# ZhenlongYuan/TSAR-MVS

Hardware: AMD Instinct MI355X
Metric: depthmap Mpixels/sec (ETH3D full-res, 8 iters) (higher is better)
Workload: dtype f32

## Files before the change

tsar-mvs_amd/csrc/pm_core.h:

```cpp
#pragma once
#include <type_traits>

#include "tsar_device_math.h"

#define PM_BLOCK 256
#define PM_RW 32

#include "pm_tap_common.h"

template <bool QUAD, bool DIFF = false>
DEVFN float sample_bilinear(const DevView& vw, int w, int h, int qpitch, float u, float v, bool q8 = false) {
    u = fminf(fmaxf(u, -1.0f), (float)w);
    v = fminf(fmaxf(v, -1.0f), (float)h);
    const float fu = floorf(u), fv = floorf(v);
    float ax = u - fu, ay = v - fv;
    if (q8) { ax = rintf(ax * 256.0f) * 0.00390625f; ay = rintf(ay * 256.0f) * 0.00390625f; }
    const int iu = (int)fu, iv = (int)fv;
    float t00, t10, t01, t11;
    if (QUAD) {
        const uint32_t off = (uint32_t)(__mul24(iv + 1, qpitch) + iu + 1) * 4u;
        const uint32_t q = *(global_u32_ptr)((const char __attribute__((address_space(1)))*)vw.quad + off);
        t00 = (float)(q & 0xffu);
        t10 = (float)((q >> 8) & 0xffu);
        t01 = (float)((q >> 16) & 0xffu);
// ... 102 lines not shown
    const int w = sc->w, h = sc->h;
    const float xf = (float)x, yf = (float)y;
    const float xd = xf * D, yd = yf * D;
    const float a = ((vw.A[0] * xd + vw.A[1] * yd) + vw.A[2] * D) + vw.b[0];
    const float b = ((vw.A[3] * xd + vw.A[4] * yd) + vw.A[5] * D) + vw.b[1];
    const float s = ((vw.A[6] * xd + vw.A[7] * yd) + vw.A[8] * D) + vw.b[2];
    float u, v;
    persp_divide_exact<true>(a, b, s, u, v);
    const float cf = floorf(u + 0.5f), rf = floorf(v + 0.5f);
    const bool inside = s > 0.0f && cf >= 0.0f && cf <= (float)(w - 1) && rf >= 0.0f && rf <= (float)(h - 1);
    float Dv = 0.0f;
    if (inside) Dv = ((global_f32_ptr)dm)[(int)rf * w + (int)cf];
    const float* M = sc->geom_back[vi];
    const float cd = cf * Dv, rd = rf * Dv;
    const float p0 = ((M[0] * cd + M[1] * rd) + M[2] * Dv) + M[3];
    const float p1 = ((M[4] * cd + M[5] * rd) + M[6] * Dv) + M[7];
    const float p2 = ((M[8] * cd + M[9] * rd) + M[10] * Dv) + M[11];
    float xq, yq;
    persp_divide_exact<true>(p0, p1, p2, xq, yq);
    const float dx = xq - xf, dy = yq - yf;
    const float e2 = dx * dx + dy * dy;
    const float tau = sc->geom_clip;
    const float r = sqrt_rsq_exact(fminf(fmaxf(e2, 0x1p-100f), 0x1p100f));
    float e = e2 < 0x1p-100f ? 0.0f : r;
    e = (inside && Dv > 0.0f && p2 > 0.0f && e2 < sc->geom_clip_sq) ? fminf(e, tau) : tau;
    return sc->geom_weight * e;
}

DEVFN float add_prior_term(const DevScene* __restrict__ sc, int x, int y, const float4& n4, float D, float c) {
    const float4* pp = sc->prior;
    if (pp == nullptr) return c;
    typedef float prior_entry __attribute__((ext_vector_type(4)));
    const prior_entry q = ((const __attribute__((address_space(1))) prior_entry*)pp)[y * sc->w + x];
    const float Dp = q.w;
    const float a = fabsf(D - Dp);
    const float rel = a / Dp;
    const float dclip = sc->prior_depth_clip, nclip = sc->prior_normal_clip;
    const float r_d = rel < dclip ? rel / dclip : 1.0f;
    const float s = 1.0f - ((n4.x * q.x + n4.y * q.y) + n4.z * q.z);
    const float s0 = s < 0.0f ? 0.0f : s;
    const float r_n = s < nclip ? s0 / nclip : 1.0f;
    const float t = (sc->prior_weight_depth * r_d) + (sc->prior_weight_normal * r_n);
    return Dp > 0.0f ? c + t : c;
}

template <int NB, int HR, bool STRICT, bool QUAD, int V = 0, int BLK = PM_BLOCK>
DEVFN float multiview_cost(const DevScene* __restrict__ sc, const typename TileOf<QUAD>::type* tile, int tw, int own, const float* wts, const PixelRef& pr,
                           int x, int y, const float4& n4, int& beview, float& ratio, bool prune = false, float cost_now = 0.0f, int* skipped = nullptr) {
    constexpr bool GEOM = (V & TSAR_V_GEOM) != 0;
    constexpr bool PRUNE = (V & TSAR_V_PRUNE) != 0;
    static_assert(!PRUNE || !GEOM, "the bound speaks of the photometric cost alone");
    constexpr bool PAIR = (V & TSAR_V_PAIR) != 0;
    static_assert(!PAIR || (!PRUNE && !GEOM), "the paired gathers exist for the plain fast box-11 kernels");
    constexpr int VT = V & ~(TSAR_V_GEOM | TSAR_V_REDRAW | TSAR_V_PRUNE | TSAR_V_PAIR);
    float best[NB];
#pragma unroll
    for (int k = 0; k < NB; k++) best[k] = __builtin_inff();
    const int num = sc->n_sel;
    int valid = 0, bv = -1;
    float cmin = __builtin_inff();
    float depth_h = 0.0f;
    if constexpr (GEOM) depth_h = plane_depth(sc->ref, n4, x, y);
    int vi_next = sc->sel[0];
    for (int i = 0; i < num; i++) {
        const int vi = vi_next;
        vi_next = sc->sel[i + 1 < num ? i + 1 : i];
        float c;
        if constexpr ((VT & TSAR_V_LUT) != 0) c = view_cost_lut<STRICT, (VT >> 11) & 7, (VT & TSAR_V_BUF) != 0 && !STRICT, (VT & TSAR_V_MIX) != 0 && !STRICT>(sc, sc->view[vi], tile, tw, own, wts, pr, x, y, n4);
        else if constexpr (QUAD && HR == 5 && r5_production_variant(VT) && PRUNE) {
            static_assert((VT & 250) == 250 && !STRICT, "pruning instantiations exist for the fast row-wise loop");
            ViewPrune vp;
            vp.on = prune; vp.skipped = false;
            vp.cost_now = cmin < cost_now ? TSAR_MAXCOST : cost_now;
            c = view_cost_r5<false, true, true, (VT & TSAR_V_BUF) != 0, (VT & TSAR_V_MIX) != 0, BLK, 0, true>(sc, sc->view[vi], tile, tw, own, wts, pr, x, y, n4, &vp);
            if (vp.skipped) *skipped += 1;
        } else if constexpr (QUAD && HR == 5 && PAIR && VT == 250) {
            static_assert(!STRICT, "the paired gathers exist for the fast row-wise loop");
            c = view_cost_r5<false, true, true, false, false, BLK, 0, false, true>(sc, sc->view[vi], tile, tw, own, wts, pr, x, y, n4);
        } else if constexpr (QUAD && HR == 5 && r5_production_variant(VT))
            c = view_cost_r5<STRICT, (VT & 128) != 0 && !STRICT, (VT & 8) != 0, (VT & TSAR_V_BUF) != 0, (VT & TSAR_V_MIX) != 0, BLK>(sc, sc->view[vi], tile, tw, own, wts, pr, x, y, n4);
#ifdef TSAR_EXPERIMENTS
        else if constexpr (QUAD && HR == 5 && PAIR && VT == (250 | 4194304))
            c = view_cost_r5<false, true, true, false, false, BLK, 3, false, true>(sc, sc->view[vi], tile, tw, own, wts, pr, x, y, n4);
        else if constexpr (QUAD && HR == 5 && r5_diag_variant(VT))
            c = view_cost_r5<false, true, true, true, true, BLK, (VT & 4194304) ? 1 : 2>(sc, sc->view[vi], tile, tw, own, wts, pr, x, y, n4);
#endif
        else {
            static_assert(VT == 0, "unknown tap-loop variant");
            c = view_cost_generic<HR, STRICT, QUAD, BLK>(sc, sc->view[vi], tile, tw, own, wts, pr, x, y, n4);
        }
        auto vmin = [](float a, float b) { float r; asm("v_min_f32 %0, %1, %2" : "=v"(r) : "v"(a), "v"(b)); return r; };
        auto vmax = [](float a, float b) { float r; asm("v_max_f32 %0, %1, %2" : "=v"(r) : "v"(a), "v"(b)); return r; };
        c = vmin(c, TSAR_MAXCOST);
        valid -= (int32_t)__float_as_uint(c - TSAR_MAXCOST) >> 31;
        if constexpr (GEOM) c = c + geom_term(sc, sc->view[vi], vi, x, y, depth_h);
        {
            const uint32_t worse = (uint32_t)((int32_t)__float_as_uint(cmin - c) >> 31);
            asm("v_bfi_b32 %0, %1, %2, %3" : "=v"(bv) : "v"(worse), "v"(bv), "s"(vi));
            cmin = vmin(cmin, c);
        }
        float v = c;
#pragma unroll
        for (int k = 0; k < NB; k++) {
            const float lo = vmin(best[k], v), hi = vmax(best[k], v);
            best[k] = lo;
            v = hi;
        }
    }
    int nb = valid;
    if (sc->cost_comb == TSAR_COMB_BEST_N) nb = min(nb, sc->n_best);
    if (nb <= 0) { beview = -1; ratio = 0.f; return TSAR_MAXCOST; }
    float cost = 0.f;
#pragma unroll
    for (int k = 0; k < NB; k++)
        if (k < nb) cost += best[k];
    cost = cost / (float)nb;
    ratio = num >= 2 ? best[0] / best[1] : 0.f;
    beview = bv;
    if constexpr (GEOM) cost = add_prior_term(sc, x, y, n4, depth_h, cost);
    return cost;
}

DEVFN void strip_tile(int t, int tiles_x, int tiles_y, int sw, int& tx, int& ty) {
    if (sw <= 0) { ty = t / tiles_x; tx = t - ty * tiles_x; return; }
    const int per_strip = sw * tiles_y;
    const int strip = t / per_strip, within = t - strip * per_strip;
    const int width = min(sw, tiles_x - strip * sw);
    ty = within / width;
    tx = strip * sw + within - ty * width;
}

static inline int strip_width(int requested, int tiles_x) {
    if (requested >= 0) return requested;
// ... 10 lines not shown
```

tsar-mvs_amd/csrc/pm_sweep.hip:

```cpp
#include "pm_sweep_impl.h"

__global__ void d16_probe_kernel(uint32_t* out) {
    __shared__ unsigned short t[64];
    t[threadIdx.x] = (unsigned short)(0x4300u + threadIdx.x);
    __syncthreads();
    uint32_t r = 0xffffffffu;
    const uint32_t addr = (uint32_t)(uintptr_t)(const __attribute__((address_space(3))) unsigned short*)(t + threadIdx.x);
    asm volatile("ds_read_u16_d16_hi %0, %1\n\ts_waitcnt lgkmcnt(0)" : "+v"(r) : "v"(addr));
    out[threadIdx.x] = r;
}
bool probe_d16_hi_zeroes(tsar_ctx* ctx) {
    CallFrame f(ctx, "d16 probe", nullptr, false);
    uint32_t h[64];
    uint32_t* d = f.out(h, 64, TSAR_MEM_HOST);
    if (f.ok()) {
        hipLaunchKernelGGL(d16_probe_kernel, dim3(1), dim3(64), 0, ctx->stream, d);
        f.launched();
    }
    bool ok = f.finish() == TSAR_OK;
    for (int i = 0; ok && i < 64; i++) ok = h[i] == ((0x4300u + i) << 16);
    return ok;
}

template <int NB, int HR>
static int launch_sweep_nh(tsar_ctx* ctx, int colour, const PlaneBuf& a, const PlaneBuf& b, const PlaneBuf& c, uint32_t sid, int dp, int dr) {
    const bool strict = ctx->hscene.flags & TSAR_FLAG_STRICT_DIV, quad = ctx->hscene.use_quad;
    const bool buf = ctx->buffer_gather && ctx->sweeps_done >= (strict ? (ctx->buffer_from > 2 ? ctx->buffer_from : 2) : ctx->buffer_from);
    const int v = ctx->variant;
    if constexpr ((NB == 2 || NB == 4) && HR == 5)
    if (quad && !(ctx->hscene.flags & TSAR_FLAG_TEX_FILTER_8BIT) && (v == 250 || v == 122 || (v == 114 && NB == 2))) {
#define SWEEP_R5(S, V, B) (buf ? launch_sweep_g<NB, 5, S, true, (V) | TSAR_V_BUF, B>(ctx, colour, a, b, c, sid, dp, dr) : launch_sweep_g<NB, 5, S, true, V, B>(ctx, colour, a, b, c, sid, dp, dr))
        const bool mix = buf && !strict && v == 250 && ctx->hscene.n_sel > 0 && ctx->hscene.view[ctx->hscene.sel[0]].dquad != nullptr;
#define SWEEP_R5_FAST250_ALL(B) (mix ? launch_sweep_g<NB, 5, false, true, 250 | TSAR_V_BUF | TSAR_V_MIX, B>(ctx, colour, a, b, c, sid, dp, dr) : SWEEP_R5(false, 250, B))
        const bool prune = NB == 2 && !strict && v == 250 && ctx->prune && ctx->prune_steps > 0 && dr && ctx->call_launch >= ctx->prune_from &&
                           ctx->hscene.cost_comb == TSAR_COMB_BEST_N && ctx->hscene.n_best == 1 && !scene_has_terms(ctx->hscene);
#define SWEEP_R5_PRUNE(B) (mix ? launch_sweep_t<2, 5, false, true, 250 | TSAR_V_BUF | TSAR_V_MIX | TSAR_V_PRUNE, B>(ctx, colour, a, b, c, sid, dp, dr) \
                           : buf ? launch_sweep_t<2, 5, false, true, 250 | TSAR_V_BUF | TSAR_V_PRUNE, B>(ctx, colour, a, b, c, sid, dp, dr)              \
                                 : launch_sweep_t<2, 5, false, true, 250 | TSAR_V_PRUNE, B>(ctx, colour, a, b, c, sid, dp, dr))
        const bool pair = NB == 2 && !strict && v == 250 && !buf && !prune && (ctx->pair & 2) && !scene_has_terms(ctx->hscene);
#define SWEEP_R5_FAST250(B) (prune ? SWEEP_R5_PRUNE(B) : pair ? launch_pm_sweep_pair(ctx, B, colour, a, b, c, sid, dp, dr) : SWEEP_R5_FAST250_ALL(B))
        if constexpr (NB == 2) {
            const int tiles256 = ((ctx->hscene.w + PM_RW - 1) / PM_RW) * ((ctx->hscene.h + 15) / 16);
            bool small = tiles256 < SWEEP_SMALL_IMAGE_TILES;
            if (ctx->force_block) small = ctx->force_block == 128;
            if (small && v != 114) {
                if (strict) return SWEEP_R5(true, 122, 128);
                return v == 250 ? SWEEP_R5_FAST250(128) : launch_sweep_g<2, 5, false, true, 122, 128>(ctx, colour, a, b, c, sid, dp, dr);
            }
            if (v == 114) return strict ? launch_sweep_g<2, 5, true, true, 114>(ctx, colour, a, b, c, sid, dp, dr) : launch_sweep_g<2, 5, false, true, 114>(ctx, colour, a, b, c, sid, dp, dr);
        }
        if (strict) return SWEEP_R5(true, 122, PM_BLOCK);
        return v == 250 ? SWEEP_R5_FAST250(PM_BLOCK) : launch_sweep_g<NB, 5, false, true, 122>(ctx, colour, a, b, c, sid, dp, dr);
#undef SWEEP_R5_FAST250
#undef SWEEP_R5_PRUNE
#undef SWEEP_R5_FAST250_ALL
#undef SWEEP_R5
    }
    constexpr int NBG = NB == 4 ? 32 : NB;
    if (strict) return quad ? launch_sweep_g<NBG, HR, true, true>(ctx, colour, a, b, c, sid, dp, dr) : launch_sweep_g<NBG, HR, true, false>(ctx, colour, a, b, c, sid, dp, dr);
    return quad ? launch_sweep_g<NBG, HR, false, true>(ctx, colour, a, b, c, sid, dp, dr) : launch_sweep_g<NBG, HR, false, false>(ctx, colour, a, b, c, sid, dp, dr);
}

int launch_pm_sweep(tsar_ctx* ctx, int colour, const PlaneBuf& same_in, const PlaneBuf& other, const PlaneBuf& same_out, uint32_t stream_id,
                    int do_prop, int do_refine) {
    const DevScene& hs = ctx->hscene;
#ifdef TSAR_EXPERIMENTS
    if (!scene_has_terms(hs)) {
        int launched = 0;
        const int rc = launch_pm_sweep_experiment(ctx, colour, same_in, other, same_out, stream_id, do_prop, do_refine, &launched);
        if (rc != TSAR_OK || launched) return rc;
    }
#endif
    const int need = views_in_cost(hs);
    const bool r5 = hs.hrad == 5 && hs.vrad == 5;
    const bool own_loop = r5 && need <= 4 && (need <= 2 || ctx->variant == 250 || ctx->variant == 122) && !(hs.flags & TSAR_FLAG_TEX_FILTER_8BIT);
    if (lut_path_applies(ctx) && (!own_loop || lut_path_forced(ctx))) return launch_pm_sweep_lut(ctx, colour, same_in, other, same_out, stream_id, do_prop, do_refine);
    if (need <= 4 && need > 2 && r5) return launch_sweep_nh<4, 5>(ctx, colour, same_in, other, same_out, stream_id, do_prop, do_refine);
    if (need <= 2) return r5 ? launch_sweep_nh<2, 5>(ctx, colour, same_in, other, same_out, stream_id, do_prop, do_refine)
                             : launch_sweep_nh<2, 0>(ctx, colour, same_in, other, same_out, stream_id, do_prop, do_refine);
    return r5 ? launch_sweep_nh<32, 5>(ctx, colour, same_in, other, same_out, stream_id, do_prop, do_refine)
              : launch_sweep_nh<32, 0>(ctx, colour, same_in, other, same_out, stream_id, do_prop, do_refine);
}
```

tsar-mvs_amd/csrc/pm_sweep_impl.h:

```cpp
#pragma once
#include "pm_dispatch.h"

#define SWEEP_SMALL_IMAGE_TILES 3072

#define CAND_SAME (1 << 30)

DEVFN void select_candidates(const DevScene* __restrict__ sc, const float* __restrict__ c_same, const float* __restrict__ c_other,
                             int x, int y, int cand[8]) {
    const int col = sc->w, row = sc->h;
    const int p = y * col + x;
    const bool fix_seed = sc->flags & TSAR_FLAG_FIX_DOWN_FAR_SEED, fix_cmp = sc->flags & TSAR_FLAG_FIX_RIGHT_FAR_CMP;
    float cmin;
    int cp, cs;
#pragma unroll
    for (int k = 0; k < 8; k++) cand[k] = -1;
    if (y > 2) {
        cp = p - 3 * col; cmin = c_other[cp];
#pragma unroll
        for (int i = 1; i < 11; ++i)
            if (y > 2 + 2 * i) { const int q = p - (3 + 2 * i) * col; const float v = c_other[q]; if (v < cmin) { cmin = v; cp = q; } }
        cand[0] = cp;
    }
    if (y < row - 3) {
        cp = p + 3 * col;
// ... 343 lines not shown
                    nt[2] = n_now.z + between(rn.u[3], -dN, dN);
                    const float inv = 1.0f / sqrtf(dot3(nt, nt));
                    nt[0] *= inv; nt[1] *= inv; nt[2] *= inv;
                    if (dot3(nt, ev) > 0.0f) { nt[0] = -nt[0]; nt[1] = -nt[1]; nt[2] = -nt[2]; }
                    n_t.x = nt[0]; n_t.y = nt[1]; n_t.z = nt[2];
                    n_t.w = plane_offset(rf, nt, ex, ey, depth_t);
                }
            }
            const float* ewts = LUTW ? wts_base : wts_base + etid;
            int bv = -1;
            float rt = 0.f, cost_t = TSAR_MAXCOST;
            if (go) cost_t = pruned_cost<NB, HR, STRICT, QUAD, V, BLK>(sc, tile, tw, eown, ewts, epr, ex, ey, n_t, bv, rt, it - trips, cost_now, memo.prune_steps, memo.prune_counts);
            if (it < trips) {
                arms_of_trip(lo, [&](int a, int j, bool has) {
                    const float c = __int_as_float(__builtin_amdgcn_ds_bpermute((j & 63) << 2, __float_as_int(cost_t)));
                    const float r = __int_as_float(__builtin_amdgcn_ds_bpermute((j & 63) << 2, __float_as_int(rt)));
                    const int b = __builtin_amdgcn_ds_bpermute((j & 63) << 2, bv);
                    if (has && c < cost_now) {
                        cost_now = c; acc_arm = a;
                        ratio_w = r; beview_w = b;
                    }
                });
            } else if (go && cost_t < cost_now) {
                cost_now = cost_t; n_now = n_t; depth_now = depth_t;
                ratio_w = rt; beview_w = bv;
            }
        }
        {
            int mx, my, mown;
            pixel_of(my_tid(), mx, my, mown);
            if (!((flags >> 9) & 1u)) return;
            const int pp = my * w + mx;
            if (acc_arm >= 0) {
                const int ci = memo.cand[(size_t)pp * 8 + acc_arm];
                const int idx = ci & 0x3fffffff;
                n_now = (ci >> 30) ? n_same[idx] : n_other[idx];
            }
            const bool changed = cost_now < c_same[pp];
            c_out[pp] = cost_now;
            n_out[pp] = n_now;
            if (changed && !final_text) { ratio_out[pp] = ratio_w; beview_out[pp] = beview_w; }
            if (changed && memo.mode) memo.changed[pp] = memo.launch;
            return;
        }
    }
    c_out[p] = cost_now;
    n_out[p] = n_now;
    if (wrote && !final_text) { ratio_out[p] = ratio_w; beview_out[p] = beview_w; }
    if (wrote && memo.mode) memo.changed[p] = memo.launch;
}


template <int HR, bool QUAD, int V>
constexpr bool sweep_has_packed_form() { return QUAD && ((HR == 5 && r5_production_variant(V & ~(TSAR_V_GEOM | TSAR_V_PRUNE))) || (V & TSAR_V_LUT) != 0); }

template <int NB, int HR, bool STRICT, bool QUAD, int V = 0, int BLK = PM_BLOCK>
static int launch_sweep_t(tsar_ctx* ctx, int colour, const PlaneBuf& same_in, const PlaneBuf& other, const PlaneBuf& same_out,
                          uint32_t stream_id, int do_prop, int do_refine) {
    constexpr int SWEEP_RH = 2 * BLK / PM_RW;
#ifdef TSAR_EXPERIMENTS
    const size_t lds_pad = ctx->lds_pad;
#else
    constexpr size_t lds_pad = 0;
#endif
    SweepMemo memo;
    memo.cand = ctx->memo_cand; memo.seq = ctx->memo_seq; memo.changed = ctx->changed_seq;
    memo.launch = ctx->launch_seq; memo.valid_from = ctx->memo_valid_from;
    memo.mode = (ctx->memo_mode && ctx->memo_cand && ctx->cost_consistent && !ctx->final_text) ? 1 : 0;
    memo.prune_steps = ((V & TSAR_V_PRUNE) != 0 && do_refine && ctx->call_launch >= ctx->prune_from) ? ctx->prune_steps : 0;
    memo.prune_counts = (V & TSAR_V_PRUNE) != 0 ? ctx->prune_counts : nullptr;
    bool packed = false;
    if constexpr (sweep_has_packed_form<HR, QUAD, V>())
        packed = memo.mode && do_prop && ctx->compact_from >= 0 && ctx->call_launch >= ctx->compact_from;
    auto kern = pm_sweep_kernel<NB, HR, STRICT, QUAD, V, BLK, false>;
    if constexpr (sweep_has_packed_form<HR, QUAD, V>())
        if (packed) kern = pm_sweep_kernel<NB, HR, STRICT, QUAD, V, BLK, true>;
    const size_t slots = packed ? 6 * (size_t)BLK : 0;
    TapGrid g;
    if (const int rc = tap_grid(ctx, kern, SWEEP_RH, BLK, QUAD, V, lds_pad + slots, g)) return rc;
    memo.slot_off = packed ? (int)(g.lds - slots) : 0;
    {
        ScopedKernelTimer tm(ctx, (V & TSAR_V_GEOM) ? "pm_sweep_geom" : "pm_sweep");
        ScopedKernelTimer tm_packed(ctx, packed ? "pm_sweep_packed" : nullptr);
        ScopedKernelTimer tm_prune(ctx, (V & TSAR_V_PRUNE) ? "pm_sweep_prune" : nullptr);
        ScopedKernelTimer tm_pair(ctx, (V & TSAR_V_PAIR) ? "pm_sweep_pair" : nullptr);
        hipLaunchKernelGGL(kern, dim3(g.n_tiles), dim3(BLK), g.lds, ctx->stream, ctx->dscene, colour, same_in.c, same_in.n4, other.c,
                           other.n4, same_out.c, same_out.n4, ctx->ratio, ctx->beview, stream_id, do_prop, do_refine, g.tiles_x, g.n_tiles,
                           ctx->cost_consistent ? 1 : 0, strip_width(ctx->strip_w, g.tiles_x), ctx->final_text, memo);
    }
    TSAR_HIP_TRY(ctx, hipGetLastError());
    return TSAR_OK;
}

template <int NB, int HR, bool STRICT, bool QUAD, int V = 0, int BLK = PM_BLOCK>
static int launch_sweep_g(tsar_ctx* ctx, int colour, const PlaneBuf& same_in, const PlaneBuf& other, const PlaneBuf& same_out,
                          uint32_t stream_id, int do_prop, int do_refine) {
    if (scene_has_terms(ctx->hscene)) return launch_sweep_t<NB, HR, STRICT, QUAD, V | TSAR_V_GEOM, BLK>(ctx, colour, same_in, other, same_out, stream_id, do_prop, do_refine);
    return launch_sweep_t<NB, HR, STRICT, QUAD, V, BLK>(ctx, colour, same_in, other, same_out, stream_id, do_prop, do_refine);
}
```

tsar-mvs_amd/csrc/pm_tap_r5.h:

```cpp
#pragma once

#define PM_PRUNE_FIRST_LINE 2
#define PM_PRUNE_LAST_LINE 4

template <bool STRICT, bool ROW, bool D16, bool BUF, bool MIX, int BLK, int DIAG = 0, bool PRUNE = false, bool PAIR = false>
DEVFN float view_cost_r5(const DevScene* __restrict__ sc, const DevView& vw, const unsigned short* tile, int tw, int own, const float* wts,
                         const PixelRef& pr, int x, int y, const float4& n4, ViewPrune* vp = nullptr) {
    static_assert(!(STRICT && ROW), "the row-wise walk changes the summation order: fast mode only");
    static_assert(!PRUNE || (ROW && D16 && !STRICT && DIAG == 0), "the partial-window bound is written for the fast row-wise loop");
    static_assert(!MIX || (BUF && !STRICT), "the half-float difference texture serves the fast arithmetic's blend through buffer loads");
    static_assert(!PAIR || (ROW && D16 && !STRICT && !BUF && !MIX && !PRUNE), "the paired gathers are written for the plain fast row-wise loop on the byte texture");
    static_assert(DIAG != 3 || PAIR, "DIAG 3 is a form of the paired loop");
    const int w = sc->w, h = sc->h, qp = sc->quad_pitch;
    const int qorg = quad_border_bytes(qp);
    float H[9];
    if (STRICT) plane_homography(sc->ref, vw, n4, H, sc->k_sparse != 0);
    else plane_homography_fast(sc->ref, vw, n4, H);
    float sum_src = 0.f, sum_src_src = 0.f, sum_ref_src = 0.f;
    bool need_clamp;
    if (!STRICT) {
        float Xc, Yc, Zc;
        pixel_homogeneous(H, (float)x, (float)y, Xc, Yc, Zc);
        const float a = fabsf(H[0]) + fabsf(H[1]), b = fabsf(H[3]) + fabsf(H[4]), c = fabsf(H[6]) + fabsf(H[7]);
        const float Zmin = fma_(-5.0f, c, Zc);
        const float r = __builtin_amdgcn_rcpf(Zmin * Zc);
        const float r5 = 5.0f * r, rc = Zmin * r;
        const float du = fma_(a, Zc, fabsf(Xc) * c) * r5, dv = fma_(b, Zc, fabsf(Yc) * c) * r5;
        const float uc = Xc * rc, vc = Yc * rc;
        const bool inside = Zmin > 0.0f && fminf(uc - du, vc - dv) >= 1.5f && uc + du <= (float)(w - 1) - 1.5f && vc + dv <= (float)(h - 1) - 1.5f;
        need_clamp = !__all(inside);
    } else {
        bool inside = true;
        float zmin = __builtin_inff(), zmax = 0.0f;
#pragma unroll
        for (int c = 0; c < 4; c++) {
            float X, Y, Z;
            pixel_homogeneous(H, (float)(x + ((c & 1) ? 5 : -5)), (float)(y + ((c & 2) ? 5 : -5)), X, Y, Z);
            const float rz = __builtin_amdgcn_rcpf(Z);
            const float u = X * rz, v = Y * rz;
            inside = inside && Z > 0.0f && u >= 1.0f && u <= (float)(w - 1) - 1.0f && v >= 1.0f && v <= (float)(h - 1) - 1.0f;
            zmin = fminf(zmin, Z); zmax = fmaxf(zmax, Z);
        }
        const float cm = (float)(max(w, h) + 32);
        const float sz = fma_(fabsf(H[6]) + fabsf(H[7]), cm, fabsf(H[8]));
        const float sx = fma_(fabsf(H[0]) + fabsf(H[1]), cm, fabsf(H[2]));
        const float sy = fma_(fabsf(H[3]) + fabsf(H[4]), cm, fabsf(H[5]));
        inside = inside && zmin >= 3.814697265625e-06f && zmax <= 131072.0f && sz * cm <= 524288.0f * zmin && fmaxf(sx, sy) <= 262144.0f * zmin;
        need_clamp = !__all(inside);
    }
    uint32_t qb_lo = 0, qb_hi = 0;
    u32x4s rsrc = {0u, 0u, 0u, 0u};
    if (!BUF) pin_quad_base(quad_origin<false>(vw, qorg), qb_lo, qb_hi);
    else rsrc = quad_descriptor<MIX>(quad_origin<MIX>(vw, qorg), h + 1, qp);
    typedef float f32x2 __attribute__((ext_vector_type(2)));
    auto line6 = [&](int i, auto clamp_tag, auto unr_tag) {
        constexpr bool CLAMP = decltype(clamp_tag)::value;
        constexpr bool UNR = decltype(unr_tag)::value;
        static_assert(!UNR || (ROW && D16), "the unrolled form is written for the row-wise walk with D16 window loads");
        const float xi = (float)((ROW ? y : x) + i);
        float bx, by, bz;
// ... 74 lines not shown
                if (jj == 1) asm("s_waitcnt vmcnt(4)" : "+v"(q[1]), "+v"(sum_src_src) : "v"(q[5]));
                if (jj == 2) asm("s_waitcnt vmcnt(3)" : "+v"(q[2]), "+v"(sum_src_src) : "v"(q[5]));
                if (jj == 3) asm("s_waitcnt vmcnt(2)" : "+v"(q[3]), "+v"(sum_src_src) : "v"(q[5]));
                if (jj == 4) asm("s_waitcnt vmcnt(1)" : "+v"(q[4]), "+v"(sum_src_src) : "v"(q[5]));
                if (jj == 5) asm("s_waitcnt vmcnt(0)" : "+v"(q[5]), "+v"(sum_src_src));
            }
            if constexpr (PAIR) {
                if ((jj & 1) == 0) q[jj] = wide[jj >> 1].x;
                else {
                    const uint32_t k = (uint32_t)(linv[jj] - linv[jj - 1]);
                    if (DIAG == 3 || k <= 3u) q[jj] = pick_dword(wide[jj >> 1], k);
                }
            }
            float s;
            if (MIX) s = blend_dquad(q2[jj], ax[jj], ay[jj]);
            else s = blend_quad<!STRICT>(q[jj], ax[jj], ay[jj]);
            if (jj == 0 && DIAG != 2) {
                if (D16)
                    asm("s_waitcnt lgkmcnt(0)" : "+v"(rcol[0]), "+v"(rcol[1]), "+v"(rcol[2]), "+v"(rcol[3]), "+v"(rcol[4]), "+v"(rcol[5]),
                        "+v"(wcol[0]), "+v"(wcol[1]), "+v"(wcol[2]), "+v"(s));
                else
                    asm("s_waitcnt lgkmcnt(0)" : "+v"(wcol[0]), "+v"(wcol[1]), "+v"(wcol[2]), "+v"(s));
            }
            const float r = D16 ? rcol[jj] : tile_value(ROW ? tile[own + i * tw + (2 * jj - 5)] : tile[own + (2 * jj - 5) * tw + i]);
            const float wt = wcol[jj >> 1][jj & 1];
            const TapSums t = tap_accumulate<STRICT>(TapSums{sum_src, sum_src_src, sum_ref_src}, wt, r, s);
            sum_src = t.src; sum_src_src = t.src_src; sum_ref_src = t.ref_src;
        }
    };
    auto pruned = [&](int line) {
        if constexpr (PRUNE) {
            if (vp->on && line >= PM_PRUNE_FIRST_LINE - 1 && line < PM_PRUNE_LAST_LINE) {
                float pa_w = 0.f, pa_r = 0.f, pa_rr = 0.f;
#pragma unroll 1
                for (int l = 0; l <= line; l++) {
#pragma unroll
                    for (int jj = 0; jj < 6; jj++) {
                        const float wt = wts[(6 * jj + l) * BLK], r = tile_value(tile[own + (2 * l - 5) * tw + (2 * jj - 5)]);
                        const float wr = wt * r;
                        pa_w += wt;
                        pa_r += wr;
                        pa_rr = fma_(wr, r, pa_rr);
                    }
                }
                if (__all(prune_proven(TapSums{sum_src, sum_src_src, sum_ref_src}, pa_w, pa_r, pa_rr, pr, vp->cost_now))) { vp->skipped = true; return true; }
            }
        }
        return false;
    };
    if (need_clamp) {
#pragma unroll 1
        for (int i = -5; i <= 5; i += 2) { line6(i, std::true_type(), std::false_type()); if (pruned((i + 5) >> 1)) return TSAR_MAXCOST; }
    } else if (MIX && !(PRUNE && vp->on)) {
#pragma unroll
        for (int i = -5; i <= 5; i += 2) line6(i, std::false_type(), std::bool_constant<MIX>());
    } else {
#pragma unroll 1
        for (int i = -5; i <= 5; i += 2) { line6(i, std::false_type(), std::false_type()); if (pruned((i + 5) >> 1)) return TSAR_MAXCOST; }
    }
    return ncc_cost(pr, TapSums{sum_src, sum_src_src, sum_ref_src});
}

__host__ __device__ constexpr bool r5_diag_variant(int V) { return V == (250 | TSAR_V_BUF | TSAR_V_MIX | 4194304) || V == (250 | TSAR_V_BUF | TSAR_V_MIX | 8388608); }
__host__ __device__ constexpr bool r5_production_variant(int V) { return V == 114 || V == 122 || V == 250 || V == (114 | TSAR_V_BUF) || V == (122 | TSAR_V_BUF) || V == (250 | TSAR_V_BUF) || V == (250 | TSAR_V_BUF | TSAR_V_MIX); }
```

tsar-mvs_amd/csrc/tsar_api.hip:

```cpp
#include <float.h>
#include <math.h>
#include <stdio.h>
#include <stdlib.h>
#include <string.h>

#include <algorithm>

#include "tsar_dev.h"

ScopedKernelTimer::ScopedKernelTimer(tsar_ctx* c, const char* name) : ctx(c) {
    if (!ctx->timing || !name) return;
    for (size_t k = 0; k < ctx->timers.size(); k++)
        if (ctx->timers[k].name == name) ti = (int)k;
    if (ti < 0) {
        ctx->timers.emplace_back();
        ctx->timers.back().name = name;
        ti = (int)ctx->timers.size() - 1;
    }
    if (hipEventCreate(&e0) != hipSuccess) { ti = -1; return; }
    if (hipEventCreate(&e1) != hipSuccess) { hipEventDestroy(e0); ti = -1; return; }
    hipEventRecord(e0, ctx->stream);
}
ScopedKernelTimer::~ScopedKernelTimer() {
    if (ti < 0) return;
// ... 129 lines not shown
    sc.n_best = p.n_best;
    sc.cost_comb = p.cost_comb;
    sc.flags = p.flags;
    sc.seed_lo = (uint32_t)p.seed;
    sc.seed_hi = (uint32_t)(p.seed >> 32);
    sc.lut_row_major = (p.flags & TSAR_FLAG_STRICT_DIV) ? 0 : 1;
    std::vector<int> d2;
    for (int i = -sc.hrad; i <= sc.hrad; i += 2)
        for (int j = -sc.vrad; j <= sc.vrad; j += 2) d2.push_back(i * i + j * j);
    std::sort(d2.begin(), d2.end());
    d2.erase(std::unique(d2.begin(), d2.end()), d2.end());
    sc.lut_classes = (int)d2.size() <= TSAR_LUT_MAX_CLASSES ? (int)d2.size() : 0;
    for (int k = 0; k < sc.lut_classes; k++) sc.lut_d2[k] = d2[k];
    const int rl = sc.lut_row_major ? sc.vrad : sc.hrad, rt = sc.lut_row_major ? sc.hrad : sc.vrad;
    sc.lut_chunk = lut_chunk_taps(rt + 1);
    sc.lut_pad_taps = (rt + sc.lut_chunk) / sc.lut_chunk * sc.lut_chunk;
    for (uint32_t& r : sc.tap_row) r = (uint32_t)sc.lut_classes * 1024u;
    for (int l = 0; l <= rl && sc.lut_classes; l++)
        for (int t = 0; t <= rt; t++) {
            const int a = 2 * l - rl, b = 2 * t - rt;
            sc.tap_row[l * sc.lut_pad_taps + t] = 1024u * (uint32_t)(std::lower_bound(d2.begin(), d2.end(), a * a + b * b) - d2.begin());
        }
}
static int upload_scene(tsar_ctx* ctx) {
    if (!ctx->dscene) TRY(dev_alloc(ctx, &ctx->dscene, 1));
    TSAR_HIP_TRY(ctx, hipMemcpyAsync(ctx->dscene, &ctx->hscene, sizeof(DevScene), hipMemcpyHostToDevice, ctx->stream));
    TSAR_HIP_TRY(ctx, hipStreamSynchronize(ctx->stream));
    return TSAR_OK;
}

extern "C" const char* tsar_version(void) {
#ifdef TSAR_EXPERIMENTS
    return "tsar-mvs_amd 0.2.0 (gfx950) +experiments";
#else
    return "tsar-mvs_amd 0.2.0 (gfx950)";
#endif
}

static void read_knobs(tsar_ctx* ctx) {
    auto num = [](const char* name, int dflt) { const char* e = getenv(name); return e && e[0] ? atoi(e) : dflt; };
    auto on = [](const char* name, bool dflt) { const char* e = getenv(name); return e && e[0] ? e[0] != '0' : dflt; };
    ctx->variant = num("TSAR_VARIANT", ctx->variant);
    ctx->buffer_gather = on("TSAR_BUFFER_GATHER", true);
    ctx->mix_gather = on("TSAR_MIX_GATHER", true);
    ctx->strip_w = num("TSAR_STRIP", -1);
    ctx->buffer_from = num("TSAR_BUFFER_FROM", 1);
    ctx->force_block = num("TSAR_BLOCK", 0);
    ctx->memo_mode = num("TSAR_MEMO", 1);
    ctx->compact_from = num("TSAR_COMPACT_FROM", 6);
    ctx->prune = num("TSAR_PRUNE", 1);
    ctx->prune_steps = std::min(std::max(num("TSAR_PRUNE_STEPS", 2), 0), 8);
    ctx->prune_from = num("TSAR_PRUNE_FROM", 1);
    ctx->pair = num("TSAR_PAIR", 3);
    ctx->lut_mode = num("TSAR_LUT", 1);
    ctx->ransac_wgs = num("TSAR_RANSAC_WGS", 8);
    ctx->ransac_chain = num("TSAR_RANSAC_CHAIN", 8);
    ctx->ransac_lookahead = num("TSAR_RANSAC_LOOKAHEAD", 0);
    ctx->ransac_poll_limit = num("TSAR_RANSAC_POLL_LIMIT", 1 << 15);
    ctx->ransac_cooperative = on("TSAR_RANSAC_COOPERATIVE", true);
    ctx->ransac_force_fallback = on("TSAR_RANSAC_FORCE_FALLBACK", false);
    ctx->render_skip = on("TSAR_RENDER_SKIP", true);
    ctx->trace_host = getenv("TSAR_TRACE_HOST") != nullptr;
#ifdef TSAR_EXPERIMENTS
    ctx->lds_pad = (size_t)num("TSAR_LDS_PAD", 0);
#endif
}

extern "C" int tsar_create(int device, tsar_ctx** out) {
    if (!out) return TSAR_ERR_INVALID;
    *out = nullptr;
    int n = 0;
    if (hipGetDeviceCount(&n) != hipSuccess || n <= 0) return TSAR_ERR_HIP;
    if (device < 0 || device >= n) return TSAR_ERR_INVALID;
    if (hipSetDevice(device) != hipSuccess) return TSAR_ERR_HIP;
    tsar_ctx* ctx = new (std::nothrow) tsar_ctx();
    if (!ctx) return TSAR_ERR_NOMEM;
    ctx->device = device;
    if (hipStreamCreateWithFlags(&ctx->stream, hipStreamNonBlocking) != hipSuccess) { delete ctx; return TSAR_ERR_HIP; }
    tsar_default_params(&ctx->params);
    ctx->variant = probe_d16_hi_zeroes(ctx) ? 250 : 114;
    read_knobs(ctx);
    *out = ctx;
    return TSAR_OK;
}

static void free_views(tsar_ctx* ctx) {
    for (auto& p : ctx->img) dev_free(p);
    for (auto& p : ctx->quad) dev_free(p);
    for (auto& p : ctx->dquad) dev_free(p);
    ctx->img.clear();
    ctx->quad.clear();
    ctx->dquad.clear();
}
static void free_geom(tsar_ctx* ctx) {
    for (auto& p : ctx->geom_maps) dev_free(p);
    ctx->geom_maps.clear();
    for (auto& p : ctx->hscene.geom_depth) p = nullptr;
    ctx->hscene.geom_on = 0;
}
static void free_prior(tsar_ctx* ctx) {
    dev_free(ctx->prior);
    ctx->hscene.prior = nullptr;
}
static void free_planes(tsar_ctx* ctx) {
    for (int b = 0; b < 2; b++) { dev_free(ctx->buf[b].c); dev_free(ctx->buf[b].n4); }
    dev_free(ctx->ratio); dev_free(ctx->depth); dev_free(ctx->scale); dev_free(ctx->lrdiff); dev_free(ctx->confid);
// ... 1258 lines not shown
```

tsar-mvs_amd/csrc/tsar_dev.h:

```cpp
#pragma once
#include <hip/hip_runtime.h>
#include <stdint.h>
#include <stdio.h>
#include <stdlib.h>

#include <chrono>
#include <string>
#include <vector>

#include "../../include/tsar.h"

#define TSAR_LUT_LINES 32
#define TSAR_LUT_TAPS 40
#define TSAR_LUT_MAX_CLASSES 144
#define TSAR_MAX_SELECTED 32

struct DevView {
    float K[9];
    float R[9];
    float t[3];
    float t_abs_lo;
    float A[9];
    float b[3];
    float t_abs_hi;
    const float* img;
    const uint32_t* quad;
    const uint2* dquad;
};

struct DevRef {
    float K[9];
    float Kinv[9];
    float Minv[9];
    float Rorig[9];
    float RorigInv[9];
    float P34[3];
    float C[3];
    float fx, f, alpha, baseline, depthMin, depthMax;
};

struct DevScene {
    int w, h;
    int n_sel;
    int hrad, vrad;
    int n_best, cost_comb;
    int refine_steps;
    int quad_pitch;
    int use_quad;
    float min_disp, max_disp;
    uint32_t flags;
    uint32_t seed_lo, seed_hi;
    int k_sparse;
    DevRef ref;
    int sel[TSAR_MAX_VIEWS];
    DevView view[TSAR_MAX_VIEWS];
    int lut_classes;
    int lut_row_major;
    int lut_chunk;
    int lut_pad_taps;
    int lut_d2[TSAR_LUT_MAX_CLASSES];
    uint32_t tap_row[TSAR_LUT_LINES * TSAR_LUT_TAPS + 8];
    const float* geom_depth[TSAR_MAX_VIEWS];
    float geom_back[TSAR_MAX_VIEWS][12];
    float geom_weight, geom_clip, geom_clip_sq;
    int geom_on;
    const float4* prior;
    float prior_weight_depth, prior_weight_normal, prior_depth_clip, prior_normal_clip;
};
static inline bool scene_has_terms(const DevScene& s) { return s.geom_on != 0 || s.prior != nullptr; }

#define TSAR_V_LUT 1024
#define TSAR_V_BUF 131072
#define TSAR_V_MIX 2097152
#define TSAR_V_GEOM 16777216
#define TSAR_V_PRUNE 67108864
#define TSAR_V_PAIR 134217728
#define TSAR_V_REDRAW 33554432

struct PlaneBuf {
    float* c;
    float4* n4;
};

struct KernelTimer {
    std::string name;
    int launches = 0;
    float total_ms = 0.f;
    std::vector<std::pair<hipEvent_t, hipEvent_t>> pending;
};

struct ScratchArena {
    char* base = nullptr;
    size_t cap = 0;
    size_t wanted = 0;
};

struct tsar_ctx {
    int device = 0;
    hipStream_t stream = nullptr;
    std::string err;
    tsar_params params{};
    bool have_params = false, have_views = false, have_state = false;
    int w = 0, h = 0, n_views = 0;
    DevScene hscene{};
    DevScene* dscene = nullptr;
    std::vector<float*> img;
    std::vector<uint32_t*> quad;
    std::vector<uint2*> dquad;
    PlaneBuf buf[2]{};
    float *ratio = nullptr, *depth = nullptr, *scale = nullptr, *lrdiff = nullptr, *confid = nullptr, *fakedepth = nullptr;
    int32_t *beview = nullptr, *canny = nullptr;
    float4* out4 = nullptr;
    bool have_out = false;
    bool cost_consistent = false;
    int n_regions = 0;
    float *region_text = nullptr, *region_size = nullptr;
    float4* region_n4 = nullptr;
    int exact_sqrt_probe = 0;
    int exact_div_probe = 0;
    int sweeps_done = 0;
    int32_t* memo_cand = nullptr;
    uint32_t* memo_seq = nullptr;
    uint32_t* changed_seq = nullptr;
    uint32_t launch_seq = 0;
    uint32_t memo_valid_from = 1;
    int call_launch = 0;
    int memo_mode = 1;
    int compact_from = 6;
    int prune = 1;
    int prune_steps = 2;
    int prune_from = 1;
    int pair = 3;
    uint32_t* prune_counts = nullptr;
    std::vector<tsar_camera> cams;
    bool views_u8 = false;
    float4* resize4 = nullptr;
    bool have_resize = false;
    const float* final_text = nullptr;
    std::vector<float*> geom_maps;
    float4* prior = nullptr;
    int variant = 2;
    bool mix_gather = true;
    bool buffer_gather = true;
    int strip_w = -1;
    int buffer_from = 1;
    int force_block = 0;
    int lut_mode = 1;
    int ransac_wgs = 8;
    int ransac_chain = 8;
    int ransac_lookahead = 0;
    int ransac_poll_limit = 1 << 15;
    bool ransac_cooperative = true;
    bool ransac_force_fallback = false;
    bool trace_host = false;
    bool render_skip = true;
#ifdef TSAR_EXPERIMENTS
    size_t lds_pad = 0;
#endif
    bool timing = false;
    std::vector<KernelTimer> timers;
    ScratchArena scratch;

    void state_scored(bool consistent) { have_state = true; have_out = false; sweeps_done = 0; cost_consistent = consistent; }
    void state_given() { have_state = true; have_out = false; cost_consistent = false; }
    void costs_voided() { cost_consistent = false; }
    void result_computed() { have_out = true; }
    void result_voided() { have_out = false; }
    void views_reset() { have_views = have_state = have_out = have_resize = false; }
};

static inline int fail(tsar_ctx* ctx, int code, const char* msg) { if (ctx) ctx->err = msg; return code; }
static inline int enter_ctx(tsar_ctx* ctx) {
    if (!ctx) return TSAR_ERR_INVALID;
    if (hipSetDevice(ctx->device) != hipSuccess) return fail(ctx, TSAR_ERR_HIP, "hipSetDevice failed");
    return TSAR_OK;
}
#define CHECK_CTX(ctx) TRY(enter_ctx(ctx))
#define NEED_VIEWS(ctx) if (!(ctx)->have_views) return fail(ctx, TSAR_ERR_STATE, "tsar_set_views has not been called")
#define NEED_SOURCES(ctx) if ((ctx)->hscene.n_sel < 1) return fail(ctx, TSAR_ERR_STATE, "no source views: tsar_set_views was given the reference view only")
#define NEED_STATE(ctx) if (!(ctx)->have_state) return fail(ctx, TSAR_ERR_STATE, "no plane state: call tsar_pm_init, tsar_load_planes or tsar_set_plane first")
#define NEED_REGIONS(ctx) if ((ctx)->n_regions < 1) return fail(ctx, TSAR_ERR_STATE, "tsar_set_regions has not been called")
#define TRY(expr) do { int rc_ = (expr); if (rc_ != TSAR_OK) return rc_; } while (0)

template <typename T>
static int dev_alloc(tsar_ctx* ctx, T** p, size_t n) {
// ... 107 lines not shown
        if (!tag) return;
        hipStreamSynchronize(ctx->stream);
        const auto n = std::chrono::steady_clock::now();
        fprintf(stderr, "%s %s %.3f ms\n", tag, what, std::chrono::duration<double, std::milli>(n - t0).count());
        t0 = n;
    }
    int finish() {
        if (!closed)
            for (const Back& b : back) copy(b.dst, b.src, b.bytes, hipMemcpyDeviceToHost);
        close();
        return rc;
    }
    void close() {
        if (closed) return;
        closed = true;
        const hipError_t e = hipStreamSynchronize(ctx->stream);
        hip(e, "hipStreamSynchronize");
        scratch.release();
    }
};

#define TSAR_HIP_TRY(ctx, expr)                                                                       \
    do {                                                                                              \
        hipError_t e_ = (expr);                                                                       \
        if (e_ != hipSuccess) {                                                                       \
            (ctx)->err = std::string(#expr) + ": " + hipGetErrorString(e_);                           \
            return TSAR_ERR_HIP;                                                                      \
        }                                                                                             \
    } while (0)

static inline int install_regions(tsar_ctx* ctx, int n) {
    ctx->n_regions = 0;
    TRY(dev_alloc(ctx, &ctx->region_text, (size_t)n));
    TRY(dev_alloc(ctx, &ctx->region_size, (size_t)n));
    TRY(dev_alloc(ctx, &ctx->region_n4, (size_t)n));
    TSAR_HIP_TRY(ctx, hipMemsetAsync(ctx->region_n4, 0, (size_t)n * 16, ctx->stream));
    return TSAR_OK;
}

struct ScopedKernelTimer {
    tsar_ctx* ctx;
    int ti = -1;
    hipEvent_t e0 = nullptr, e1 = nullptr;
    ScopedKernelTimer(tsar_ctx* c, const char* name);
    ~ScopedKernelTimer();
};

int launch_build_quad(tsar_ctx* ctx, const float* img, uint32_t* quad, int w, int h, int* nonintegral_flag);
int launch_expand_u8(tsar_ctx* ctx, const uint8_t* in, float* out, size_t n);
int launch_build_dquad(tsar_ctx* ctx, const uint32_t* quad, uint2* dquad, int w, int h);
int launch_pm_init(tsar_ctx* ctx);
int launch_pm_init_pair(tsar_ctx* ctx);
int launch_pm_sweep_pair(tsar_ctx* ctx, int block, int colour, const PlaneBuf& same_in, const PlaneBuf& other, const PlaneBuf& same_out,
                         uint32_t stream_id, int do_prop, int do_refine);
bool probe_d16_hi_zeroes(tsar_ctx* ctx);
int launch_pm_sweep(tsar_ctx* ctx, int colour, const PlaneBuf& same_in, const PlaneBuf& other, const PlaneBuf& same_out,
                    uint32_t stream_id, int do_prop, int do_refine);
int launch_pm_sweep_lut(tsar_ctx* ctx, int colour, const PlaneBuf& same_in, const PlaneBuf& other, const PlaneBuf& same_out, uint32_t stream_id,
                        int do_prop, int do_refine);
int launch_pm_full_lut(tsar_ctx* ctx, bool init, bool redraw, const float4* planes, float* c, float4* n, int32_t* bv, float* rt);
int lut_chunk_taps(int taps_per_line);
static inline bool lut_path_forced(const tsar_ctx* ctx) { return ctx->lut_mode == 2; }
static inline bool lut_path_applies(const tsar_ctx* ctx) {
    const bool off = ctx->lut_mode == 0;
    const DevScene& hs = ctx->hscene;
    const bool d16_ok = (hs.flags & TSAR_FLAG_STRICT_DIV) || (ctx->variant & 8);
    return !off && d16_ok && hs.use_quad && hs.lut_classes > 0;
}
int launch_pm_sweep_experiment(tsar_ctx* ctx, int colour, const PlaneBuf& same_in, const PlaneBuf& other, const PlaneBuf& same_out, uint32_t stream_id,
                               int do_prop, int do_refine, int* launched);
int launch_pm_cost_planes(tsar_ctx* ctx, const float4* planes, float* cost, int32_t* beview, float* ratio);
int launch_pm_rescore(tsar_ctx* ctx, const float4* planes, float* cost, float4* n, int32_t* beview, float* ratio);
int launch_pm_upsample(tsar_ctx* ctx, const float4* coarse, int cw, int ch);
int launch_pm_upsample_merge(tsar_ctx* ctx, const float4* coarse, int cw, int ch);
int launch_pm_upsample_lut(tsar_ctx* ctx, bool merge, const float4* coarse, int cw, int ch);
int launch_pyr_down(tsar_ctx* ctx, const float* src, int w, int h, void* dst, bool u8);
int launch_geom_pyramid(tsar_ctx* ctx, const float* src, int w, int h, float* dst);
int launch_pyramid_planes(tsar_ctx* ctx, const float4* src, int w, int h, float4* dst);
int launch_geom_check(tsar_ctx* ctx, const float* depth, int depth_stride, const tsar_geom_check_params* p, uint8_t* count_out,
                      float* depth_out);
int launch_geom_reproject(tsar_ctx* ctx, const tsar_geom_reproject_params* p, uint32_t* zbuf, unsigned long long* mask, float* depth_out,
                          uint8_t* count_out);
int launch_merge_candidates(tsar_ctx* ctx, const float* depth, float4* cand);
int launch_merge_select(tsar_ctx* ctx, const float4* cand, const float* cand_c, const int32_t* cand_bv, const float* cand_rt,
                        unsigned long long* n_taken);
int launch_get_disp(tsar_ctx* ctx, const float* depth_in, const float* normal_world);
int launch_plane_prior(tsar_ctx* ctx, const float* depth_in, const float* normal_world, float4* prior);
size_t plane_prior_build_grid_keys(int w, int h, int cell, int max_levels);
int launch_plane_prior_build(tsar_ctx* ctx, const float* depth, const float* score, int cell, int max_levels, unsigned long long* grid,
                             float* depth_out, float* normal_out, uint8_t* level_out);
int run_cloud_distance(CallFrame& f, const float* query, long long n_query, int query_stride, const float* target, long long n_target, int target_stride,
                       float r2, double edge, long long max_pairs, int n_tol, const float* tol2, float* dist2_out, int32_t* index_out, int64_t* within_out,
                       int64_t* n_valid_out, int64_t* pairs_out);
int run_cloud_voxels(CallFrame& f, const float* cloud, long long n, int stride, double voxel, const float* dist2, int n_tol, const float* tol2, int32_t* rank_out,
                     long long cap, int32_t* rep_out, int32_t* count_out, int32_t* within_out, int64_t* n_voxels_out, int64_t* n_valid_out,
                     int mem);
struct CrViewHost { float P[12]; float fr; int max_px, w, h; bool foot; };
int run_cloud_render(CallFrame& f, const float* cloud, long long n, int stride, const CrViewHost& vh, float occlusion_diff, float depth_diff, int min_points,
                     long long max_splats, float* depth_out, uint8_t* count_out, int32_t* index_out,
                     int64_t* n_splats_out);
int run_depth_compare(CallFrame& f, const float* depth, const float* gt, const uint8_t* mask, long long n, int n_tol, const float* tol, float* error_out,
                      unsigned long long* counters_out);
int launch_compute_disp(tsar_ctx* ctx);
int launch_compute_disp_final(tsar_ctx* ctx, const float4* resize4, const float* text);
int launch_depth_to_plane(tsar_ctx* ctx);
int launch_getview(tsar_ctx* ctx);
// ... 10 lines not shown
```

Baseline: 51.11.

## Add software-pipelined ring of in-flight gathers for the difference-texture box-11 walk

Adds a RING variant of the 11x11 tap cost loop. It keeps six buffer gathers in flight at once and issues the next row's gather as each tap is consumed, using explicit vmcnt/lgkmcnt waits, sched barriers and raised wave priority. The reference pixels and weights are read from LDS once per line. The aim is to hide global gather latency behind the blend and accumulate arithmetic. The cost is hand-scheduled inline asm and higher register pressure. The variant is enabled by default from sweep 3 onward for NB=2 mixed-gather scenes without extra terms.

```diff
diff --git a/tsar-mvs_amd/csrc/pm_core.h b/tsar-mvs_amd/csrc/pm_core.h
--- a/tsar-mvs_amd/csrc/pm_core.h
+++ b/tsar-mvs_amd/csrc/pm_core.h
@@ -178,7 +178,9 @@
     static_assert(!PRUNE || !GEOM, "the bound speaks of the photometric cost alone");
     constexpr bool PAIR = (V & TSAR_V_PAIR) != 0;
     static_assert(!PAIR || (!PRUNE && !GEOM), "the paired gathers exist for the plain fast box-11 kernels");
-    constexpr int VT = V & ~(TSAR_V_GEOM | TSAR_V_REDRAW | TSAR_V_PRUNE | TSAR_V_PAIR);
+    constexpr bool RING = (V & TSAR_V_RING) != 0;
+    constexpr int VT = V & ~(TSAR_V_GEOM | TSAR_V_REDRAW | TSAR_V_PRUNE | TSAR_V_PAIR | TSAR_V_RING);
+    static_assert(!RING || (VT == (250 | TSAR_V_BUF | TSAR_V_MIX) && !GEOM && !PAIR && !STRICT && QUAD && HR == 5), "the ring exists for the fast difference-texture box-11 kernels");
     float best[NB];
 #pragma unroll
     for (int k = 0; k < NB; k++) best[k] = __builtin_inff();
@@ -198,13 +200,13 @@
             ViewPrune vp;
             vp.on = prune; vp.skipped = false;
             vp.cost_now = cmin < cost_now ? TSAR_MAXCOST : cost_now;
-            c = view_cost_r5<false, true, true, (VT & TSAR_V_BUF) != 0, (VT & TSAR_V_MIX) != 0, BLK, 0, true>(sc, sc->view[vi], tile, tw, own, wts, pr, x, y, n4, &vp);
+            c = view_cost_r5<false, true, true, (VT & TSAR_V_BUF) != 0, (VT & TSAR_V_MIX) != 0, BLK, 0, true, false, RING>(sc, sc->view[vi], tile, tw, own, wts, pr, x, y, n4, &vp);
             if (vp.skipped) *skipped += 1;
         } else if constexpr (QUAD && HR == 5 && PAIR && VT == 250) {
             static_assert(!STRICT, "the paired gathers exist for the fast row-wise loop");
             c = view_cost_r5<false, true, true, false, false, BLK, 0, false, true>(sc, sc->view[vi], tile, tw, own, wts, pr, x, y, n4);
         } else if constexpr (QUAD && HR == 5 && r5_production_variant(VT))
-            c = view_cost_r5<STRICT, (VT & 128) != 0 && !STRICT, (VT & 8) != 0, (VT & TSAR_V_BUF) != 0, (VT & TSAR_V_MIX) != 0, BLK>(sc, sc->view[vi], tile, tw, own, wts, pr, x, y, n4);
+            c = view_cost_r5<STRICT, (VT & 128) != 0 && !STRICT, (VT & 8) != 0, (VT & TSAR_V_BUF) != 0, (VT & TSAR_V_MIX) != 0, BLK, 0, false, false, RING>(sc, sc->view[vi], tile, tw, own, wts, pr, x, y, n4);
 #ifdef TSAR_EXPERIMENTS
         else if constexpr (QUAD && HR == 5 && PAIR && VT == (250 | 4194304))
             c = view_cost_r5<false, true, true, false, false, BLK, 3, false, true>(sc, sc->view[vi], tile, tw, own, wts, pr, x, y, n4);
diff --git a/tsar-mvs_amd/csrc/pm_ring.hip b/tsar-mvs_amd/csrc/pm_ring.hip
--- /dev/null
+++ b/tsar-mvs_amd/csrc/pm_ring.hip
@@ -0,0 +1,12 @@
+#include "pm_sweep_impl.h"
+
+int launch_pm_sweep_ring(tsar_ctx* ctx, int block, bool prune, int colour, const PlaneBuf& same_in, const PlaneBuf& other, const PlaneBuf& same_out,
+                         uint32_t stream_id, int do_prop, int do_refine) {
+    constexpr int V = 250 | TSAR_V_BUF | TSAR_V_MIX | TSAR_V_RING;
+    if (prune) {
+        if (block == 128) return launch_sweep_t<2, 5, false, true, V | TSAR_V_PRUNE, 128>(ctx, colour, same_in, other, same_out, stream_id, do_prop, do_refine);
+        return launch_sweep_t<2, 5, false, true, V | TSAR_V_PRUNE, PM_BLOCK>(ctx, colour, same_in, other, same_out, stream_id, do_prop, do_refine);
+    }
+    if (block == 128) return launch_sweep_t<2, 5, false, true, V, 128>(ctx, colour, same_in, other, same_out, stream_id, do_prop, do_refine);
+    return launch_sweep_t<2, 5, false, true, V, PM_BLOCK>(ctx, colour, same_in, other, same_out, stream_id, do_prop, do_refine);
+}
diff --git a/tsar-mvs_amd/csrc/pm_sweep.hip b/tsar-mvs_amd/csrc/pm_sweep.hip
--- a/tsar-mvs_amd/csrc/pm_sweep.hip
+++ b/tsar-mvs_amd/csrc/pm_sweep.hip
@@ -38,7 +38,8 @@
                            : buf ? launch_sweep_t<2, 5, false, true, 250 | TSAR_V_BUF | TSAR_V_PRUNE, B>(ctx, colour, a, b, c, sid, dp, dr)              \
                                  : launch_sweep_t<2, 5, false, true, 250 | TSAR_V_PRUNE, B>(ctx, colour, a, b, c, sid, dp, dr))
         const bool pair = NB == 2 && !strict && v == 250 && !buf && !prune && (ctx->pair & 2) && !scene_has_terms(ctx->hscene);
-#define SWEEP_R5_FAST250(B) (prune ? SWEEP_R5_PRUNE(B) : pair ? launch_pm_sweep_pair(ctx, B, colour, a, b, c, sid, dp, dr) : SWEEP_R5_FAST250_ALL(B))
+        const bool ring = NB == 2 && mix && ctx->ring > 0 && ctx->sweeps_done >= ctx->ring && !scene_has_terms(ctx->hscene);
+#define SWEEP_R5_FAST250(B) (ring ? launch_pm_sweep_ring(ctx, B, prune, colour, a, b, c, sid, dp, dr) : prune ? SWEEP_R5_PRUNE(B) : pair ? launch_pm_sweep_pair(ctx, B, colour, a, b, c, sid, dp, dr) : SWEEP_R5_FAST250_ALL(B))
         if constexpr (NB == 2) {
             const int tiles256 = ((ctx->hscene.w + PM_RW - 1) / PM_RW) * ((ctx->hscene.h + 15) / 16);
             bool small = tiles256 < SWEEP_SMALL_IMAGE_TILES;
diff --git a/tsar-mvs_amd/csrc/pm_sweep_impl.h b/tsar-mvs_amd/csrc/pm_sweep_impl.h
--- a/tsar-mvs_amd/csrc/pm_sweep_impl.h
+++ b/tsar-mvs_amd/csrc/pm_sweep_impl.h
@@ -419,7 +419,7 @@
 
 
 template <int HR, bool QUAD, int V>
-constexpr bool sweep_has_packed_form() { return QUAD && ((HR == 5 && r5_production_variant(V & ~(TSAR_V_GEOM | TSAR_V_PRUNE))) || (V & TSAR_V_LUT) != 0); }
+constexpr bool sweep_has_packed_form() { return QUAD && ((HR == 5 && r5_production_variant(V & ~(TSAR_V_GEOM | TSAR_V_PRUNE | TSAR_V_RING))) || (V & TSAR_V_LUT) != 0); }
 
 template <int NB, int HR, bool STRICT, bool QUAD, int V = 0, int BLK = PM_BLOCK>
 static int launch_sweep_t(tsar_ctx* ctx, int colour, const PlaneBuf& same_in, const PlaneBuf& other, const PlaneBuf& same_out,
@@ -451,6 +451,7 @@
         ScopedKernelTimer tm_packed(ctx, packed ? "pm_sweep_packed" : nullptr);
         ScopedKernelTimer tm_prune(ctx, (V & TSAR_V_PRUNE) ? "pm_sweep_prune" : nullptr);
         ScopedKernelTimer tm_pair(ctx, (V & TSAR_V_PAIR) ? "pm_sweep_pair" : nullptr);
+        ScopedKernelTimer tm_ring(ctx, (V & TSAR_V_RING) ? "pm_sweep_ring" : nullptr);
         hipLaunchKernelGGL(kern, dim3(g.n_tiles), dim3(BLK), g.lds, ctx->stream, ctx->dscene, colour, same_in.c, same_in.n4, other.c,
                            other.n4, same_out.c, same_out.n4, ctx->ratio, ctx->beview, stream_id, do_prop, do_refine, g.tiles_x, g.n_tiles,
                            ctx->cost_consistent ? 1 : 0, strip_width(ctx->strip_w, g.tiles_x), ctx->final_text, memo);
diff --git a/tsar-mvs_amd/csrc/pm_tap_r5.h b/tsar-mvs_amd/csrc/pm_tap_r5.h
--- a/tsar-mvs_amd/csrc/pm_tap_r5.h
+++ b/tsar-mvs_amd/csrc/pm_tap_r5.h
@@ -3,9 +3,10 @@
 #define PM_PRUNE_FIRST_LINE 2
 #define PM_PRUNE_LAST_LINE 4
 
-template <bool STRICT, bool ROW, bool D16, bool BUF, bool MIX, int BLK, int DIAG = 0, bool PRUNE = false, bool PAIR = false>
+template <bool STRICT, bool ROW, bool D16, bool BUF, bool MIX, int BLK, int DIAG = 0, bool PRUNE = false, bool PAIR = false, bool RING = false>
 DEVFN float view_cost_r5(const DevScene* __restrict__ sc, const DevView& vw, const unsigned short* tile, int tw, int own, const float* wts,
                          const PixelRef& pr, int x, int y, const float4& n4, ViewPrune* vp = nullptr) {
+    static_assert(!RING || (MIX && ROW && D16 && DIAG == 0 && !PAIR), "the ring is a form of the unrolled difference-texture walk");
     static_assert(!(STRICT && ROW), "the row-wise walk changes the summation order: fast mode only");
     static_assert(!PRUNE || (ROW && D16 && !STRICT && DIAG == 0), "the partial-window bound is written for the fast row-wise loop");
     static_assert(!MIX || (BUF && !STRICT), "the half-float difference texture serves the fast arithmetic's blend through buffer loads");
@@ -186,8 +187,61 @@
 #pragma unroll 1
         for (int i = -5; i <= 5; i += 2) { line6(i, std::true_type(), std::false_type()); if (pruned((i + 5) >> 1)) return TSAR_MAXCOST; }
     } else if (MIX && !(PRUNE && vp->on)) {
-#pragma unroll
-        for (int i = -5; i <= 5; i += 2) line6(i, std::false_type(), std::bool_constant<MIX>());
+        if constexpr (RING) {
+            constexpr int U = BLK / 64;
+            const float uhi = (float)(w - 1), vhi = (float)(h - 1);
+            const uint32_t wa = (uint32_t)(uintptr_t)(const __attribute__((address_space(3))) float*)wts;
+            const uint32_t a0 = (uint32_t)(uintptr_t)(const __attribute__((address_space(3))) unsigned short*)(tile + own - 5 * tw - 5);
+            float bx, by, bz, ax[6], ay[6], rcol[6];
+            f32x2 wcol[3];
+            uint64_t q2[6];
+            __builtin_amdgcn_s_setprio(2);
+            tap_line_base<false, true>(H, (float)(y - 5), bx, by, bz);
+#pragma unroll
+            for (int jj = 0; jj < 6; jj++) {
+                float X, Y, Z;
+                int lin;
+                tap_homogeneous<false, true>(H, (float)(x + 2 * jj - 5), bx, by, bz, X, Y, Z);
+                tap_position<false, false>(X, Y, Z, uhi, vhi, qp, ax[jj], ay[jj], lin);
+                q2[jj] = buffer_gather<true>(lin, rsrc);
+            }
+            __builtin_amdgcn_sched_barrier(0);
+#pragma unroll
+            for (int t = 0; t < 36; t++) {
+                const int line = t / 6, jj = t % 6;
+                if (jj == 0) {
+                    const float dep = line == 0 ? bz : sum_ref_src;
+#pragma unroll
+                    for (int k = 0; k < 3; k++)
+                        asm("ds_read2st64_b32 %0, %1 offset0:%2 offset1:%3" : "=v"(wcol[k]) : "v"(wa), "n"(2 * U * 6 * k + U * line), "n"(2 * U * 6 * k + U * 6 + U * line), "v"(dep));
+#pragma unroll
+                    for (int k = 0; k < 6; k++)
+                        asm("ds_read_u16_d16_hi %0, %1 offset:%2" : "=v"(rcol[k]) : "v"(a0), "n"(k * 4 + line * 2 * (PM_RW + 10) * 2), "v"(dep));
+                }
+                if (t == 0) asm("s_waitcnt vmcnt(5)" : "+v"(q2[0]) : "v"(q2[5]));
+                else if (t < 35) asm("s_waitcnt vmcnt(%2)" : "+v"(q2[jj]), "+v"(sum_src_src) : "n"(t < 30 ? 5 : 35 - t), "v"(q2[t < 30 ? (jj + 5) % 6 : 5]));
+                else asm("s_waitcnt vmcnt(0)" : "+v"(q2[5]), "+v"(sum_src_src));
+                float s = blend_dquad(q2[jj], ax[jj], ay[jj]);
+                if (jj == 0)
+                    asm("s_waitcnt lgkmcnt(0)" : "+v"(rcol[0]), "+v"(rcol[1]), "+v"(rcol[2]), "+v"(rcol[3]), "+v"(rcol[4]), "+v"(rcol[5]),
+                        "+v"(wcol[0]), "+v"(wcol[1]), "+v"(wcol[2]), "+v"(s));
+                const TapSums ts = tap_accumulate<false>(TapSums{sum_src, sum_src_src, sum_ref_src}, wcol[jj >> 1][jj & 1], rcol[jj], s);
+                sum_src = ts.src; sum_src_src = ts.src_src; sum_ref_src = ts.ref_src;
+                if (t < 30) {
+                    if (jj == 0) tap_line_base<false, true>(H, (float)(y + 2 * (line + 1) - 5), bx, by, bz);
+                    float X, Y, Z;
+                    int lin;
+                    tap_homogeneous<false, true>(H, (float)(x + 2 * jj - 5), bx, by, bz, X, Y, Z);
+                    tap_position<false, false>(X, Y, Z, uhi, vhi, qp, ax[jj], ay[jj], lin);
+                    q2[jj] = buffer_gather<true>(lin, rsrc);
+                }
+                __builtin_amdgcn_sched_barrier(0);
+            }
+            __builtin_amdgcn_s_setprio(0);
+        } else {
+#pragma unroll
+            for (int i = -5; i <= 5; i += 2) line6(i, std::false_type(), std::bool_constant<MIX>());
+        }
     } else {
 #pragma unroll 1
         for (int i = -5; i <= 5; i += 2) { line6(i, std::false_type(), std::false_type()); if (pruned((i + 5) >> 1)) return TSAR_MAXCOST; }
diff --git a/tsar-mvs_amd/csrc/tsar_api.hip b/tsar-mvs_amd/csrc/tsar_api.hip
--- a/tsar-mvs_amd/csrc/tsar_api.hip
+++ b/tsar-mvs_amd/csrc/tsar_api.hip
@@ -205,6 +205,7 @@
     ctx->prune_steps = std::min(std::max(num("TSAR_PRUNE_STEPS", 2), 0), 8);
     ctx->prune_from = num("TSAR_PRUNE_FROM", 1);
     ctx->pair = num("TSAR_PAIR", 3);
+    ctx->ring = num("TSAR_RING", ctx->ring);
     ctx->lut_mode = num("TSAR_LUT", 1);
     ctx->ransac_wgs = num("TSAR_RANSAC_WGS", 8);
     ctx->ransac_chain = num("TSAR_RANSAC_CHAIN", 8);
diff --git a/tsar-mvs_amd/csrc/tsar_dev.h b/tsar-mvs_amd/csrc/tsar_dev.h
--- a/tsar-mvs_amd/csrc/tsar_dev.h
+++ b/tsar-mvs_amd/csrc/tsar_dev.h
@@ -75,6 +75,7 @@
 #define TSAR_V_GEOM 16777216
 #define TSAR_V_PRUNE 67108864
 #define TSAR_V_PAIR 134217728
+#define TSAR_V_RING 268435456
 #define TSAR_V_REDRAW 33554432
 
 struct PlaneBuf {
@@ -131,6 +132,7 @@
     int prune_steps = 2;
     int prune_from = 1;
     int pair = 3;
+    int ring = 3;
     uint32_t* prune_counts = nullptr;
     std::vector<tsar_camera> cams;
     bool views_u8 = false;
@@ -344,6 +346,8 @@
 int launch_pm_init(tsar_ctx* ctx);
 int launch_pm_init_pair(tsar_ctx* ctx);
 int launch_pm_sweep_pair(tsar_ctx* ctx, int block, int colour, const PlaneBuf& same_in, const PlaneBuf& other, const PlaneBuf& same_out,
+                         uint32_t stream_id, int do_prop, int do_refine);
+int launch_pm_sweep_ring(tsar_ctx* ctx, int block, bool prune, int colour, const PlaneBuf& same_in, const PlaneBuf& other, const PlaneBuf& same_out,
                          uint32_t stream_id, int do_prop, int do_refine);
 bool probe_d16_hi_zeroes(tsar_ctx* ctx);
 int launch_pm_sweep(tsar_ctx* ctx, int colour, const PlaneBuf& same_in, const PlaneBuf& other, const PlaneBuf& same_out,
```

Result: faster. 52.05 (median of 6 runs) (+1.8%).
